# Yeicor/sdf-viewer

Measured on AMD Instinct MI355X. Metric: Mvoxels/s grid fill + Mrays/s sphere-trace @1080p, demo SDF, higher is better.
Workload: dtype f32

## Files before the change

### profiles/r02/raymarch_loop_hand.s

```
s_mov_b64 s[76:77], exec
s_and_b64 exec, exec, s[2:3]
s_cbranch_execz .Ldone_2
v_mov_b32 v40, v9
v_mov_b32 v42, v14
v_mov_b32 v43, v15
v_mov_b32 v44, v1
v_mov_b32 v46, v2
v_mov_b32 v47, v3
s_mov_b32 s66, s5
s_mov_b32 s67, s6
s_mov_b32 s70, s17
s_mov_b32 s71, s18
s_mov_b32 s72, 0xbf000000
s_mov_b32 s73, 0xbf000000
s_add_i32 s75, s40, -1
s_add_i32 s82, s19, 2
s_add_i32 s83, s19, 4
s_movk_i32 s74, 254
s_lshl_b32 s64, 1, s82
s_add_i32 s86, s23, s82
s_lshl_b32 s86, 1, s86
s_add_u32 s68, s34, s86
s_addc_u32 s69, s35, 0
s_add_u32 s64, s34, s64
s_addc_u32 s65, s35, 0
s_add_u32 s86, s64, s86
s_addc_u32 s87, s65, 0
v_mov_b32 v68, 0x7f800000
v_mov_b32 v70, 0x7f800000
v_mov_b32 v71, 0x7f800000
.Lloop_2:
v_max3_f32 v32, |v40|, |v42|, |v43|
v_subrev_f32_e32 v48, s4, v40
v_pk_add_f32 v[50:51], v[42:43], s[66:67] neg_lo:[0,1] neg_hi:[0,1]
v_mul_f32_e32 v48, s16, v48
v_pk_mul_f32 v[50:51], v[50:51], s[70:71]
v_subrev_f32_e32 v32, s7, v32
v_add_f32_e32 v48, -0.5, v48
v_pk_add_f32 v[50:51], v[50:51], s[72:73]
v_cmpx_nlt_f32_e32 vcc, 0x38d1b717, v32
s_cbranch_execz .Ldone_2
v_sub_f32_e32 v52, v48, v68
v_sub_f32_e32 v54, v50, v70
v_sub_f32_e32 v56, v51, v71
v_max3_u32 v32, v52, v54, v56
v_cmp_gt_u32_e32 vcc, 0x3f800000, v32
s_andn1_saveexec_b64 s[78:79], vcc
s_cbranch_execnz .Lfetch_2
.Lcached_2:
s_mov_b64 exec, s[78:79]
v_sub_f32_e32 v53, 1.0, v52
v_sub_f32_e32 v55, 1.0, v54
v_sub_f32_e32 v57, 1.0, v56
v_pk_mul_f32 v[34:35], v[62:63], v[52:53] op_sel_hi:[1,0]
v_pk_mul_f32 v[38:39], v[66:67], v[52:53] op_sel_hi:[1,0]
v_pk_mul_f32 v[32:33], v[60:61], v[52:53] op_sel:[0,1] op_sel_hi:[1,1]
v_pk_mul_f32 v[36:37], v[64:65], v[52:53] op_sel:[0,1] op_sel_hi:[1,1]
v_pk_add_f32 v[32:33], v[32:33], v[34:35]
v_pk_add_f32 v[36:37], v[36:37], v[38:39]
v_pk_mul_f32 v[32:33], v[32:33], v[54:55] op_sel:[0,1] op_sel_hi:[1,1]
v_pk_mul_f32 v[36:37], v[36:37], v[54:55] op_sel_hi:[1,0]
v_pk_add_f32 v[32:33], v[32:33], v[36:37]
v_pk_mul_f32 v[32:33], v[32:33], v[56:57] op_sel:[0,1] op_sel_hi:[1,0]
v_add_f32_e32 v36, v32, v33
v_add_f32_e32 v36, 0xbdcccccd, v36
v_cmpx_ngt_f32_e32 vcc, 0x3727c5ac, v36
v_mul_f32_e32 v32, v44, v36
v_pk_mul_f32 v[34:35], v[46:47], v[36:37] op_sel_hi:[1,0]
v_add_f32_e32 v40, v40, v32
v_pk_add_f32 v[42:43], v[42:43], v[34:35]
s_add_u32 s74, s74, -1
s_cbranch_scc1 .Lloop_2
s_branch .Ldone_2
.Lfetch_2:
v_floor_f32_e32 v68, v48
v_floor_f32_e32 v70, v50
v_floor_f32_e32 v71, v51
v_cvt_i32_f32_e32 v32, v68
v_cvt_i32_f32_e32 v33, v70
v_cvt_i32_f32_e32 v34, v71
v_sub_f32_e32 v52, v48, v68
v_sub_f32_e32 v54, v50, v70
v_sub_f32_e32 v56, v51, v71
v_max3_u32 v35, v32, v33, v34
v_cmp_gt_u32_e32 vcc, s28, v35
s_xor_b64 vcc, vcc, exec
s_cbranch_scc1 .Lborder_2
v_lshl_add_u32 v39, v34, s23, v33
v_lshl_add_u32 v39, v39, s19, v32
v_lshlrev_b32_e32 v39, 2, v39
global_load_dwordx2 v[24:25], v39, s[34:35]
global_load_dwordx2 v[26:27], v39, s[64:65]
global_load_dwordx2 v[28:29], v39, s[68:69]
global_load_dwordx2 v[30:31], v39, s[86:87]
s_waitcnt vmcnt(1)
v_pk_mov_b32 v[60:61], v[24:25], v[28:29] op_sel:[0,0]
v_pk_mov_b32 v[62:63], v[24:25], v[28:29] op_sel:[1,1]
s_waitcnt vmcnt(0)
v_pk_mov_b32 v[64:65], v[26:27], v[30:31] op_sel:[0,0]
v_pk_mov_b32 v[66:67], v[26:27], v[30:31] op_sel:[1,1]
s_branch .Lcached_2
.Lborder_2:
v_max_i32_e32 v35, 0, v32
v_max_i32_e32 v37, 0, v33
v_max_i32_e32 v38, 0, v34
v_add_u32_e32 v32, 1, v32
v_add_u32_e32 v33, 1, v33
v_add_u32_e32 v34, 1, v34
v_min_i32_e32 v32, s40, v32
v_min_i32_e32 v33, s41, v33
v_min_i32_e32 v34, s42, v34
v_lshl_add_u32 v28, v38, s23, v37
v_lshl_add_u32 v29, v38, s23, v33
v_lshl_add_u32 v30, v34, s23, v37
v_lshl_add_u32 v31, v34, s23, v33
v_min_i32_e32 v36, s75, v35
v_lshlrev_b32_e32 v39, 2, v36
v_lshl_add_u32 v28, v28, s82, v39
v_lshl_add_u32 v29, v29, s82, v39
v_lshl_add_u32 v30, v30, s82, v39
v_lshl_add_u32 v31, v31, s82, v39
global_load_dwordx2 v[24:25], v28, s[34:35]
global_load_dwordx2 v[26:27], v29, s[34:35]
global_load_dwordx2 v[28:29], v30, s[34:35]
global_load_dwordx2 v[30:31], v31, s[34:35]
v_cmp_eq_u32_e64 s[80:81], v35, v36
v_add_u32_e32 v36, 1, v36
v_cmp_eq_u32_e32 vcc, v32, v36
s_waitcnt vmcnt(3)
v_cndmask_b32_e64 v60, v25, v24, s[80:81]
v_cndmask_b32_e32 v62, v24, v25, vcc
s_waitcnt vmcnt(2)
v_cndmask_b32_e64 v64, v27, v26, s[80:81]
v_cndmask_b32_e32 v66, v26, v27, vcc
s_waitcnt vmcnt(1)
v_cndmask_b32_e64 v61, v29, v28, s[80:81]
v_cndmask_b32_e32 v63, v28, v29, vcc
s_waitcnt vmcnt(0)
v_cndmask_b32_e64 v65, v31, v30, s[80:81]
v_cndmask_b32_e32 v67, v30, v31, vcc
s_branch .Lcached_2
.Ldone_2:
s_mov_b64 s[30:31], exec
s_mov_b32 s14, s74
s_and_b64 exec, s[76:77], s[2:3]
v_mov_b32 v9, v40
v_mov_b32 v14, v42
v_mov_b32 v15, v43
s_mov_b64 exec, s[76:77]
```

### sdf-viewer_amd/csrc/march_asm_loop.h

```cpp
#pragma once

#include "march_sampler.h"

namespace sdfv {
namespace {

#ifdef SDFV_TUNING
#define SDFV_MARCH_ASM_TUNE(x) x
#else
#define SDFV_MARCH_ASM_TUNE(x) ""
#endif
#define SDFV_MARCH_ASM_HEAD(ROW_BYTES)                                                                                         \
    "s_mov_b64 s[76:77], exec\n"                                                                                    \
    "s_and_b64 exec, exec, %[cov]\n"                                                                                \
    "s_cbranch_execz .Ldone_%=\n"                                                                                   \
          \
    "s_mov_b32 s66, %[miny]\n s_mov_b32 s67, %[minz]\n"                                            \
    "s_mov_b32 s70, %[ky]\n s_mov_b32 s71, %[kz]\n"                                                    \
    "s_mov_b32 s72, 0xbf000000\n s_mov_b32 s73, 0xbf000000\n"                                      \
    "s_add_i32 s75, %[wm1], -1\n"                                                                         \
    "s_lshl_b32 s82, %[w], 2\n s_lshl_b32 s83, %[w], 4\n"         \
    "s_lshl_b32 s85, %[w], 3\n"                                      \
    "s_movk_i32 s74, 254\n"                                                                      \
     \
    "s_mov_b32 s64, " ROW_BYTES "\n"                                                                                 \
    "s_mul_i32 s86, %[h], " ROW_BYTES "\n"                                                                           \
    "s_add_u32 s68, %[base_lo], s86\n s_addc_u32 s69, %[base_hi], 0\n"                                      \
    "s_add_u32 s64, %[base_lo], s64\n s_addc_u32 s65, %[base_hi], 0\n"                                      \
    "s_add_u32 s86, s64, s86\n s_addc_u32 s87, s65, 0\n"                                                    \
    SDFV_MARCH_ASM_TUNE("s_mov_b32 s84, 0\n")                  \
    "v_mov_b32 v68, 0x7f800000\n v_mov_b32 v70, 0x7f800000\n v_mov_b32 v71, 0x7f800000\n"     \
    ".Lloop_%=:\n"
#define SDFV_MARCH_ASM_OOB4_A "v_sub_f32_e64 v32, |v40|, %[mx]\n"
#define SDFV_MARCH_ASM_OOB4_B "v_sub_f32_e64 v33, |v42|, %[my]\n"
#define SDFV_MARCH_ASM_OOB4_C "v_sub_f32_e64 v34, |v43|, %[mz]\n"
#define SDFV_MARCH_ASM_OOB4_D "v_max3_f32 v32, v32, v33, v34\n"
#define SDFV_MARCH_ASM_OOB2_A "v_max3_f32 v32, |v40|, |v42|, |v43|\n"
#define SDFV_MARCH_ASM_OOB2_D "v_subrev_f32_e32 v32, %[mx], v32\n"
#define SDFV_MARCH_ASM_TOP(T_STEP, OOB_A, OOB_B, OOB_C, OOB_D)                                                      \
    OOB_A                                                                                                           \
    "v_subrev_f32_e32 v48, %[minx], v40\n"                                                                          \
    OOB_B                                                                                                           \
    "v_pk_add_f32 v[50:51], v[42:43], s[66:67] neg_lo:[0,1] neg_hi:[0,1]\n"                                         \
    OOB_C                                                                                                           \
    "v_mul_f32_e32 v48, %[kx], v48\n"                                                                               \
    "v_pk_mul_f32 v[50:51], v[50:51], s[70:71]\n"                                                                   \
    OOB_D                                                                                                           \
    "v_add_f32_e32 v48, -0.5, v48\n"                                                                                \
    "v_pk_add_f32 v[50:51], v[50:51], s[72:73]\n"                                                                   \
    "v_cmpx_nlt_f32_e32 vcc, 0x38d1b717, v32\n"                                           \
    "s_cbranch_execz .Ldone_%=\n"                                                                                   \
    "v_sub_f32_e32 v52, v48, v68\n"                                                                              \
    "v_sub_f32_e32 v54, v50, v70\n"                                                                              \
    "v_sub_f32_e32 v56, v51, v71\n" T_STEP                                                                       \
    "v_max3_u32 v32, v52, v54, v56\n"                                                                            \
    "v_cmp_gt_u32_e32 vcc, 0x3f800000, v32\n"                                                                       \
    "s_andn1_saveexec_b64 s[78:79], vcc\n"                                      \
    "s_cbranch_execnz .Lfetch_%=\n"                                  \
    ".Lcached_%=:\n"
#define SDFV_MARCH_ASM_FETCH_PREP(INTERIOR)                                                                         \
    ".Lfetch_%=:\n"                                                                                                 \
    SDFV_MARCH_ASM_TUNE("s_add_u32 s84, s84, 1\n")                                                                  \
        \
    "v_floor_f32_e32 v68, v48\n v_floor_f32_e32 v70, v50\n v_floor_f32_e32 v71, v51\n"                         \
    "v_cvt_i32_f32_e32 v32, v68\n v_cvt_i32_f32_e32 v33, v70\n v_cvt_i32_f32_e32 v34, v71\n"                      \
    "v_sub_f32_e32 v52, v48, v68\n v_sub_f32_e32 v54, v50, v70\n v_sub_f32_e32 v56, v51, v71\n"             \
     \
    "v_max3_u32 v35, v32, v33, v34\n"                                                                               \
    "v_cmp_gt_u32_e32 vcc, %[thresh], v35\n"                                                                        \
    "s_xor_b64 vcc, vcc, exec\n"                                                                                    \
    "s_cbranch_scc1 .Lborder_%=\n"                                                                                  \
    "v_mad_u32_u24 v39, v34, %[h], v33\n"                     \
    "v_mad_u32_u24 v39, v39, %[w], v32\n" INTERIOR                                                               \
    "s_branch .Lcached_%=\n"                                                                                        \
    ".Lborder_%=:\n"                                                                                                \
    "v_max_i32_e32 v35, 0, v32\n v_max_i32_e32 v37, 0, v33\n v_max_i32_e32 v38, 0, v34\n"         \
    "v_add_u32_e32 v32, 1, v32\n v_add_u32_e32 v33, 1, v33\n v_add_u32_e32 v34, 1, v34\n"                            \
    "v_min_i32_e32 v32, %[wm1], v32\n v_min_i32_e32 v33, %[hm1], v33\n v_min_i32_e32 v34, %[dm1], v34\n"   \
    "v_mad_u32_u24 v28, v38, %[h], v37\n"                                                      \
    "v_mad_u32_u24 v29, v38, %[h], v33\n"                                                      \
    "v_mad_u32_u24 v30, v34, %[h], v37\n"                                                      \
    "v_mad_u32_u24 v31, v34, %[h], v33\n"
#define SDFV_MARCH_ASM_INTERIOR_DIST                                                                                \
    "v_lshlrev_b32_e32 v39, 2, v39\n"                                                                               \
    "global_load_dwordx2 v[24:25], v39, %[base]\n"                                        \
    "global_load_dwordx2 v[26:27], v39, s[64:65]\n"                                       \
    "global_load_dwordx2 v[28:29], v39, s[68:69]\n"                                       \
    "global_load_dwordx2 v[30:31], v39, s[86:87]\n"                                       \
    "s_waitcnt vmcnt(1)\n"                                                                                          \
    "v_pk_mov_b32 v[60:61], v[24:25], v[28:29] op_sel:[0,0]\n"                                    \
    "v_pk_mov_b32 v[62:63], v[24:25], v[28:29] op_sel:[1,1]\n"                                    \
    "s_waitcnt vmcnt(0)\n"                                                                                          \
    "v_pk_mov_b32 v[64:65], v[26:27], v[30:31] op_sel:[0,0]\n"                                    \
    "v_pk_mov_b32 v[66:67], v[26:27], v[30:31] op_sel:[1,1]\n"
#define SDFV_MARCH_ASM_INTERIOR_TEX0                                                                                \
    "v_lshlrev_b32_e32 v39, 4, v39\n"                                                                               \
    "global_load_dword v60, v39, %[base]\n global_load_dword v62, v39, %[base] offset:16\n"                       \
    "global_load_dword v64, v39, s[64:65]\n global_load_dword v66, v39, s[64:65] offset:16\n"                     \
    "global_load_dword v61, v39, s[68:69]\n global_load_dword v63, v39, s[68:69] offset:16\n"                     \
    "global_load_dword v65, v39, s[86:87]\n global_load_dword v67, v39, s[86:87] offset:16\n"                     \
    "s_waitcnt vmcnt(0)\n"
#define SDFV_MARCH_ASM_INTERIOR_PAIRS                                                                               \
    "v_lshlrev_b32_e32 v39, 3, v39\n"                                                                               \
    "global_load_dwordx4 v[24:27], v39, %[base]\n"                                  \
    "global_load_dwordx4 v[28:31], v39, s[68:69]\n"                                 \
    "s_waitcnt vmcnt(0)\n"                                                                                          \
    "v_pk_mov_b32 v[60:61], v[24:25], v[28:29] op_sel:[0,0]\n"                                    \
    "v_pk_mov_b32 v[64:65], v[24:25], v[28:29] op_sel:[1,1]\n"                                    \
    "v_pk_mov_b32 v[62:63], v[26:27], v[30:31] op_sel:[0,0]\n"                                    \
    "v_pk_mov_b32 v[66:67], v[26:27], v[30:31] op_sel:[1,1]\n"
#define SDFV_MARCH_ASM_FETCH_PAIRS                                                                                  \
    "v_lshlrev_b32_e32 v35, 3, v35\n v_lshlrev_b32_e32 v32, 3, v32\n"                  \
    "v_mad_u32_u24 v24, v28, s85, v35\n v_mad_u32_u24 v25, v28, s85, v32\n"                                          \
    "global_load_dword v60, v24, %[base]\n global_load_dword v62, v25, %[base]\n"                                  \
    "v_mad_u32_u24 v26, v29, s85, v35\n v_mad_u32_u24 v27, v29, s85, v32\n"                                          \
    "global_load_dword v64, v26, %[base]\n global_load_dword v66, v27, %[base]\n"                                  \
    "v_mad_u32_u24 v24, v30, s85, v35\n v_mad_u32_u24 v25, v30, s85, v32\n"                                          \
    "global_load_dword v61, v24, %[base]\n global_load_dword v63, v25, %[base]\n"                                  \
    "v_mad_u32_u24 v26, v31, s85, v35\n v_mad_u32_u24 v27, v31, s85, v32\n"                                          \
    "global_load_dword v65, v26, %[base]\n global_load_dword v67, v27, %[base]\n"                                  \
    "s_waitcnt vmcnt(0)\n"                                                                                          \
    "s_branch .Lcached_%=\n"
#define SDFV_MARCH_ASM_INTERIOR_ILV                                                                                 \
    "s_lshr_b32 s80, %[h], 1\n"                                                                                     \
    "v_and_b32_e32 v48, 1, v33\n"                                                                  \
    "v_lshrrev_b32_e32 v35, 1, v33\n"                                                              \
    "v_add_u32_e32 v36, 1, v33\n"                                                                                   \
    "v_lshrrev_b32_e32 v36, 1, v36\n"                                                        \
    "v_mad_u32_u24 v35, v34, s80, v35\n v_mad_u32_u24 v36, v34, s80, v36\n"              \
    "v_mad_u32_u24 v35, v35, %[w], v32\n v_mad_u32_u24 v37, v36, %[w], v32\n"                                        \
    "v_lshlrev_b32_e32 v36, 3, v35\n v_lshlrev_b32_e32 v37, 3, v37\n"                                               \
    "v_cmp_eq_u32_e32 vcc, 1, v48\n"                                                                                \
    "global_load_dwordx4 v[24:27], v36, %[base]\n"                      \
    "global_load_dwordx4 v[32:35], v36, s[68:69]\n"                                                      \
    "s_and_saveexec_b64 s[80:81], vcc\n"                      \
    "global_load_dwordx3 v[28:30], v37, %[base]\n"                                   \
    "global_load_dwordx3 v[36:38], v37, s[68:69]\n"                                                      \
    "s_mov_b64 exec, s[80:81]\n"                                                                                    \
    "s_waitcnt vmcnt(2)\n"                                                                                          \
    "v_cndmask_b32_e32 v60, v24, v25, vcc\n v_cndmask_b32_e32 v62, v26, v27, vcc\n"          \
    "v_cndmask_b32_e32 v61, v32, v33, vcc\n v_cndmask_b32_e32 v63, v34, v35, vcc\n"                  \
    "s_waitcnt vmcnt(0)\n"                                                                                          \
    "v_cndmask_b32_e32 v64, v25, v28, vcc\n v_cndmask_b32_e32 v66, v27, v30, vcc\n"      \
    "v_cndmask_b32_e32 v65, v33, v36, vcc\n v_cndmask_b32_e32 v67, v35, v38, vcc\n"
#define SDFV_MARCH_ASM_ILV_ROW(R)                             \
    "v_and_b32_e32 v36, 1, v" #R "\n"                                                                     \
    "v_lshrrev_b32_e32 v" #R ", 1, v" #R "\n"                                     \
    "v_mul_u32_u24_e32 v" #R ", s85, v" #R "\n"                                                         \
    "v_lshl_add_u32 v" #R ", v36, 2, v" #R "\n"
#define SDFV_MARCH_ASM_FETCH_ILV                                                                                    \
    "v_lshlrev_b32_e32 v35, 3, v35\n v_lshlrev_b32_e32 v32, 3, v32\n"         \
    SDFV_MARCH_ASM_ILV_ROW(28) SDFV_MARCH_ASM_ILV_ROW(29) SDFV_MARCH_ASM_ILV_ROW(30) SDFV_MARCH_ASM_ILV_ROW(31)       \
    "v_add_u32_e32 v24, v28, v35\n v_add_u32_e32 v25, v28, v32\n"                                                    \
    "global_load_dword v60, v24, %[base]\n global_load_dword v62, v25, %[base]\n"                                  \
    "v_add_u32_e32 v26, v29, v35\n v_add_u32_e32 v27, v29, v32\n"                                                    \
    "global_load_dword v64, v26, %[base]\n global_load_dword v66, v27, %[base]\n"                                  \
    "v_add_u32_e32 v24, v30, v35\n v_add_u32_e32 v25, v30, v32\n"                                                    \
    "global_load_dword v61, v24, %[base]\n global_load_dword v63, v25, %[base]\n"                                  \
    "v_add_u32_e32 v26, v31, v35\n v_add_u32_e32 v27, v31, v32\n"                                                    \
    "global_load_dword v65, v26, %[base]\n global_load_dword v67, v27, %[base]\n"                                  \
    "s_waitcnt vmcnt(0)\n"                                                                                          \
    "s_branch .Lcached_%=\n"
#define SDFV_MARCH_ASM_FETCH_DIST                                                                                   \
    "v_min_i32_e32 v36, s75, v35\n"                                                         \
    "v_lshlrev_b32_e32 v39, 2, v36\n"                                                                               \
    "v_mad_u32_u24 v28, v28, s82, v39\n v_mad_u32_u24 v29, v29, s82, v39\n"                                          \
    "v_mad_u32_u24 v30, v30, s82, v39\n v_mad_u32_u24 v31, v31, s82, v39\n"                                          \
    "global_load_dwordx2 v[24:25], v28, %[base]\n"                                                     \
    "global_load_dwordx2 v[26:27], v29, %[base]\n"                                                     \
    "global_load_dwordx2 v[28:29], v30, %[base]\n"                                                     \
    "global_load_dwordx2 v[30:31], v31, %[base]\n"                                                     \
    "v_cmp_eq_u32_e64 s[80:81], v35, v36\n"                                                             \
    "v_add_u32_e32 v36, 1, v36\n"                                                                                   \
    "v_cmp_eq_u32_e32 vcc, v32, v36\n"                                                                  \
    "s_waitcnt vmcnt(3)\n"                                                                                          \
    "v_cndmask_b32_e64 v60, v25, v24, s[80:81]\n v_cndmask_b32_e32 v62, v24, v25, vcc\n"           \
    "s_waitcnt vmcnt(2)\n"                                                                                          \
    "v_cndmask_b32_e64 v64, v27, v26, s[80:81]\n v_cndmask_b32_e32 v66, v26, v27, vcc\n"           \
    "s_waitcnt vmcnt(1)\n"                                                                                          \
    "v_cndmask_b32_e64 v61, v29, v28, s[80:81]\n v_cndmask_b32_e32 v63, v28, v29, vcc\n"           \
    "s_waitcnt vmcnt(0)\n"                                                                                          \
    "v_cndmask_b32_e64 v65, v31, v30, s[80:81]\n v_cndmask_b32_e32 v67, v30, v31, vcc\n"           \
    "s_branch .Lcached_%=\n"
#define SDFV_MARCH_ASM_FETCH_TEX0                                                                                   \
    "v_lshlrev_b32_e32 v35, 4, v35\n v_lshlrev_b32_e32 v32, 4, v32\n"                  \
    "v_mad_u32_u24 v24, v28, s83, v35\n v_mad_u32_u24 v25, v28, s83, v32\n"                                          \
    "global_load_dword v60, v24, %[base]\n global_load_dword v62, v25, %[base]\n"                                  \
    "v_mad_u32_u24 v26, v29, s83, v35\n v_mad_u32_u24 v27, v29, s83, v32\n"                                          \
    "global_load_dword v64, v26, %[base]\n global_load_dword v66, v27, %[base]\n"                                  \
    "v_mad_u32_u24 v24, v30, s83, v35\n v_mad_u32_u24 v25, v30, s83, v32\n"                                          \
    "global_load_dword v61, v24, %[base]\n global_load_dword v63, v25, %[base]\n"                                  \
    "v_mad_u32_u24 v26, v31, s83, v35\n v_mad_u32_u24 v27, v31, s83, v32\n"                                          \
    "global_load_dword v65, v26, %[base]\n global_load_dword v67, v27, %[base]\n"                                  \
    "s_waitcnt vmcnt(0)\n"                                                                                          \
    "s_branch .Lcached_%=\n"
#define SDFV_MARCH_ASM_FILTER                                                                                       \
    "s_mov_b64 exec, s[78:79]\n"                                                                                    \
    "v_sub_f32_e32 v53, 1.0, v52\n v_sub_f32_e32 v55, 1.0, v54\n v_sub_f32_e32 v57, 1.0, v56\n"                \
                                                                \
    "v_pk_mul_f32 v[34:35], v[62:63], v[52:53] op_sel_hi:[1,0]\n"                                                \
    "v_pk_mul_f32 v[38:39], v[66:67], v[52:53] op_sel_hi:[1,0]\n"                                                \
    "v_pk_mul_f32 v[32:33], v[60:61], v[52:53] op_sel:[0,1] op_sel_hi:[1,1]\n"                                   \
    "v_pk_mul_f32 v[36:37], v[64:65], v[52:53] op_sel:[0,1] op_sel_hi:[1,1]\n"                                   \
    "v_pk_add_f32 v[32:33], v[32:33], v[34:35]\n"                                                    \
    "v_pk_add_f32 v[36:37], v[36:37], v[38:39]\n"                                                    \
                                                                                                   \
    "v_pk_mul_f32 v[32:33], v[32:33], v[54:55] op_sel:[0,1] op_sel_hi:[1,1]\n"                                     \
    "v_pk_mul_f32 v[36:37], v[36:37], v[54:55] op_sel_hi:[1,0]\n"                                                  \
    "v_pk_add_f32 v[32:33], v[32:33], v[36:37]\n"                                                      \
                                                                       \
    "v_pk_mul_f32 v[32:33], v[32:33], v[56:57] op_sel:[0,1] op_sel_hi:[1,0]\n"       \
    "v_add_f32_e32 v36, v32, v33\n"                                                                                 \
    "v_add_f32_e32 v36, 0xbdcccccd, v36\n"                                                                          \
                                                                                 \
    "v_cmpx_ngt_f32_e32 vcc, 0x3727c5ac, v36\n"
#define SDFV_MARCH_ASM_ADVANCE                                                                                      \
                                                           \
    "v_mul_f32_e32 v32, v44, v36\n"                                                                                \
    "v_pk_mul_f32 v[34:35], v[46:47], v[36:37] op_sel_hi:[1,0]\n"                                                  \
    "v_add_f32_e32 v40, v40, v32\n"                                                                                 \
    "v_pk_add_f32 v[42:43], v[42:43], v[34:35]\n"                                                                   \
    "s_add_u32 s74, s74, -1\n"                                                    \
    "s_cbranch_scc1 .Lloop_%=\n"                                                                                    \
    "s_branch .Ldone_%=\n"
#define SDFV_MARCH_ASM_EPILOGUE                                                                                     \
    ".Ldone_%=:\n"                                                                                                  \
    "s_mov_b64 %[ran], exec\n"                                        \
    "s_mov_b32 %[left], s74\n"                                                                                      \
    SDFV_MARCH_ASM_TUNE("s_lshl_b32 s84, s84, 16\n s_and_b32 %[left], %[left], 0xffff\n s_or_b32 %[left], %[left], s84\n") \
    "s_and_b64 exec, s[76:77], %[cov]\n"                                                                            \
    "s_nop 0\n"
#define SDFV_MARCH_ASM_END "s_mov_b64 exec, s[76:77]\n"
#define SDFV_MARCH_ASM_OPERANDS                                                                                     \
    [dx] "v"(dirx), [dy] "v"(diry), [dz] "v"(dirz), [cov] "s"(cov), [mx] "s"(a.rp.bounds_max[0]),    \
        [my] "s"(a.rp.bounds_max[1]), [mz] "s"(a.rp.bounds_max[2]), [minx] "s"(a.rp.bounds_min[0]),                 \
        [miny] "s"(a.rp.bounds_min[1]), [minz] "s"(a.rp.bounds_min[2]), [kx] "s"(kx), [ky] "s"(ky), [kz] "s"(kz),   \
        [wm1] "s"(wm1), [hm1] "s"(hm1), [dm1] "s"(dm1), [w] "s"(t.w), [h] "s"(t.h), [base] "s"(vol), [base_lo] "s"(base_lo), [base_hi] "s"(base_hi), [thresh] "s"(thresh)
#define SDFV_MARCH_ASM_CLOBBERS                                                                                     \
    "vcc", "scc", "memory", "s64", "s65", "s66", "s67", "s68", "s69", "s70", "s71", "s72", "s73", "s74", "s75",    \
        "s76", "s77", "s78", "s79", "s80", "s81", "s82", "s83", "s84", "s85", "s86", "s87", "v24", "v25", "v26", "v27", "v28",  \
        "v29", "v30", "v31", "v32", "v33", "v34", "v35", "v36", "v37", "v38", "v39", "v48", "v50", "v51", "v52",    \
        "v53", "v54", "v55", "v56", "v57", "v58", "v59", "v60", "v61", "v62", "v63", "v64", "v65", "v66", "v67", "v68",   \
        "v70", "v71"

template <int MODE, bool T>
__device__ __forceinline__ void march_asm(const RaymarchArgs& a, const Tex& t, V3 ray_dir, bool covered, V3& ray_pos,
                                          float& dist_from_origin, int& status, int& steps, int& iterations) {
    const float* __restrict__ vol = march_volume<MODE>(a);
    auto uniform = [](float f) { return __int_as_float(__builtin_amdgcn_readfirstlane(__float_as_int(f))); };
    const float kx = uniform(a.inv_bsize[0] * (float)t.w), ky = uniform(a.inv_bsize[1] * (float)t.h),
                kz = uniform(a.inv_bsize[2] * (float)t.d);
    const int wm1 = t.w - 1, hm1 = t.h - 1, dm1 = t.d - 1;
    const unsigned long long cov = __ballot(covered);
    const uint32_t base_lo = (uint32_t)(uintptr_t)vol, base_hi = (uint32_t)((uintptr_t)vol >> 32);
    const uint32_t thresh = (t.w == t.h && t.h == t.d && !a.no_interior_fetch) ? (uint32_t)t.w - 1u : 0u;
    unsigned long long ran_out;
    int left = 254;
    register float px asm("v40") = ray_pos.x;
    register float py asm("v42") = ray_pos.y;
    register float pz asm("v43") = ray_pos.z;
    register float dirx asm("v44") = ray_dir.x;
    register float diry asm("v46") = ray_dir.y;
    register float dirz asm("v47") = ray_dir.z;
#define SDFV_MARCH_ASM_OOB_BOX SDFV_MARCH_ASM_OOB4_A, SDFV_MARCH_ASM_OOB4_B, SDFV_MARCH_ASM_OOB4_C, SDFV_MARCH_ASM_OOB4_D
#define SDFV_MARCH_ASM_OOB_CUBE SDFV_MARCH_ASM_OOB2_A, "", "", SDFV_MARCH_ASM_OOB2_D
#define SDFV_MARCH_ASM_TOP_(T_STEP, ...) SDFV_MARCH_ASM_TOP(T_STEP, __VA_ARGS__)
#define SDFV_MARCH_ASM_RUN_AUX(SHIFT, INTERIOR, FETCH, OOB)                                                         \
    asm volatile("v_mov_b32 v58, %[tt]\n v_mov_b32 v59, 0\n" SDFV_MARCH_ASM_HEAD(SHIFT)                             \
                 SDFV_MARCH_ASM_TOP_("v_add_u32_e32 v59, 1, v59\n", OOB) SDFV_MARCH_ASM_FILTER                       \
                 "v_add_f32_e32 v58, v58, v36\n" SDFV_MARCH_ASM_ADVANCE SDFV_MARCH_ASM_FETCH_PREP(INTERIOR) FETCH    \
                 SDFV_MARCH_ASM_EPILOGUE "v_mov_b32 %[tt], v58\n v_mov_b32 %[n], v59\n" SDFV_MARCH_ASM_END           \
                 : [px] "+v"(px), [py] "+v"(py), [pz] "+v"(pz), [tt] "+v"(tt), [n] "+v"(n), [ran] "=&s"(ran_out),   \
                   [left] "=&s"(left)                                                                               \
                 : SDFV_MARCH_ASM_OPERANDS                                                                          \
                 : SDFV_MARCH_ASM_CLOBBERS)
#define SDFV_MARCH_ASM_RUN(SHIFT, INTERIOR, FETCH, OOB)                                                             \
    asm volatile(SDFV_MARCH_ASM_HEAD(SHIFT) SDFV_MARCH_ASM_TOP_("", OOB) SDFV_MARCH_ASM_FILTER SDFV_MARCH_ASM_ADVANCE \
                     SDFV_MARCH_ASM_FETCH_PREP(INTERIOR) FETCH SDFV_MARCH_ASM_EPILOGUE SDFV_MARCH_ASM_END            \
                 : [px] "+v"(px), [py] "+v"(py), [pz] "+v"(pz), [ran] "=&s"(ran_out), [left] "=&s"(left)            \
                 : SDFV_MARCH_ASM_OPERANDS                                                                          \
                 : SDFV_MARCH_ASM_CLOBBERS)
#define SDFV_MARCH_ASM_VOL_TEX0 "s83", SDFV_MARCH_ASM_INTERIOR_TEX0, SDFV_MARCH_ASM_FETCH_TEX0
#define SDFV_MARCH_ASM_VOL_DIST "s82", SDFV_MARCH_ASM_INTERIOR_DIST, SDFV_MARCH_ASM_FETCH_DIST
#define SDFV_MARCH_ASM_VOL_PAIRS "s85", SDFV_MARCH_ASM_INTERIOR_PAIRS, SDFV_MARCH_ASM_FETCH_PAIRS
#define SDFV_MARCH_ASM_VOL_ILV "s82", SDFV_MARCH_ASM_INTERIOR_ILV, SDFV_MARCH_ASM_FETCH_ILV
#define SDFV_MARCH_ASM_PER_BOX(RUN, ...)                                                                            \
    if (cube) RUN(__VA_ARGS__, SDFV_MARCH_ASM_OOB_CUBE);                                                            \
    else RUN(__VA_ARGS__, SDFV_MARCH_ASM_OOB_BOX)
#define SDFV_MARCH_ASM_PER_VOLUME(RUN)                                                                              \
    if (MODE == kMarchIlv) { SDFV_MARCH_ASM_PER_BOX(RUN, SDFV_MARCH_ASM_VOL_ILV); }                                 \
    else if (MODE == kMarchPairs) { SDFV_MARCH_ASM_PER_BOX(RUN, SDFV_MARCH_ASM_VOL_PAIRS); }                        \
    else if (MODE == kMarchDist) { SDFV_MARCH_ASM_PER_BOX(RUN, SDFV_MARCH_ASM_VOL_DIST); }                          \
    else { SDFV_MARCH_ASM_PER_BOX(RUN, SDFV_MARCH_ASM_VOL_TEX0); }
    const bool cube = a.cube_box != 0;
    if (T) {
        float tt = dist_from_origin;
        int n = 0;
        SDFV_MARCH_ASM_PER_VOLUME(SDFV_MARCH_ASM_RUN_AUX)
        dist_from_origin = tt;
        steps = n;
    } else {
// ... 18 lines not shown
```

Measured before the change: 204,600.

## Unroll hand-written sphere-trace loop 3x and move fetch exec masking to out-of-line blocks

The inline-asm march loop is unrolled three times, with the iteration counter cut from 254 to 84 so the total step budget stays about the same. Each copy gets its own out-of-line fetch and border block, and exit labels that reconstruct the remaining-step count when tuning is enabled. The common cached path now takes a plain vcc branch and skips the per-iteration saveexec/restore exec pair; the fetch block sets and restores exec itself. The aim is to cut loop overhead and scalar exec traffic per step, at the cost of larger code and a step budget of 252 instead of 254.

```diff
diff --git a/profiles/r02/raymarch_loop_hand.s b/profiles/r02/raymarch_loop_hand.s
--- a/profiles/r02/raymarch_loop_hand.s
+++ b/profiles/r02/raymarch_loop_hand.s
@@ -1,54 +1,120 @@
 s_mov_b64 s[76:77], exec
-s_and_b64 exec, exec, s[2:3]
-s_cbranch_execz .Ldone_2
-v_mov_b32 v40, v9
-v_mov_b32 v42, v14
-v_mov_b32 v43, v15
-v_mov_b32 v44, v1
-v_mov_b32 v46, v2
-v_mov_b32 v47, v3
+s_and_b64 exec, exec, s[12:13]
+s_cbranch_execz .Ldone_16
 s_mov_b32 s66, s5
 s_mov_b32 s67, s6
-s_mov_b32 s70, s17
-s_mov_b32 s71, s18
+s_mov_b32 s70, s23
+s_mov_b32 s71, s36
 s_mov_b32 s72, 0xbf000000
 s_mov_b32 s73, 0xbf000000
 s_add_i32 s75, s40, -1
-s_add_i32 s82, s19, 2
-s_add_i32 s83, s19, 4
-s_movk_i32 s74, 254
-s_lshl_b32 s64, 1, s82
-s_add_i32 s86, s23, s82
-s_lshl_b32 s86, 1, s86
-s_add_u32 s68, s34, s86
-s_addc_u32 s69, s35, 0
-s_add_u32 s64, s34, s64
-s_addc_u32 s65, s35, 0
+s_lshl_b32 s82, s10, 2
+s_lshl_b32 s83, s10, 4
+s_lshl_b32 s85, s10, 3
+s_movk_i32 s74, 84
+s_mov_b32 s64, s82
+s_mul_i32 s86, s38, s82
+s_add_u32 s68, s2, s86
+s_addc_u32 s69, s3, 0
+s_add_u32 s64, s2, s64
+s_addc_u32 s65, s3, 0
 s_add_u32 s86, s64, s86
 s_addc_u32 s87, s65, 0
 v_mov_b32 v68, 0x7f800000
 v_mov_b32 v70, 0x7f800000
 v_mov_b32 v71, 0x7f800000
-.Lloop_2:
+.Lloop_16:
 v_max3_f32 v32, |v40|, |v42|, |v43|
 v_subrev_f32_e32 v48, s4, v40
 v_pk_add_f32 v[50:51], v[42:43], s[66:67] neg_lo:[0,1] neg_hi:[0,1]
-v_mul_f32_e32 v48, s16, v48
+v_mul_f32_e32 v48, s22, v48
 v_pk_mul_f32 v[50:51], v[50:51], s[70:71]
 v_subrev_f32_e32 v32, s7, v32
 v_add_f32_e32 v48, -0.5, v48
 v_pk_add_f32 v[50:51], v[50:51], s[72:73]
 v_cmpx_nlt_f32_e32 vcc, 0x38d1b717, v32
-s_cbranch_execz .Ldone_2
+s_cbranch_execz .Ldone0_16
 v_sub_f32_e32 v52, v48, v68
 v_sub_f32_e32 v54, v50, v70
 v_sub_f32_e32 v56, v51, v71
 v_max3_u32 v32, v52, v54, v56
-v_cmp_gt_u32_e32 vcc, 0x3f800000, v32
-s_andn1_saveexec_b64 s[78:79], vcc
-s_cbranch_execnz .Lfetch_2
-.Lcached_2:
-s_mov_b64 exec, s[78:79]
+v_cmp_le_u32_e32 vcc, 0x3f800000, v32
+s_cbranch_vccnz .Lfetch0_16
+.Lcached0_16:
+v_sub_f32_e32 v53, 1.0, v52
+v_sub_f32_e32 v55, 1.0, v54
+v_sub_f32_e32 v57, 1.0, v56
+v_pk_mul_f32 v[34:35], v[62:63], v[52:53] op_sel_hi:[1,0]
+v_pk_mul_f32 v[38:39], v[66:67], v[52:53] op_sel_hi:[1,0]
+v_pk_mul_f32 v[32:33], v[60:61], v[52:53] op_sel:[0,1] op_sel_hi:[1,1]
+v_pk_mul_f32 v[36:37], v[64:65], v[52:53] op_sel:[0,1] op_sel_hi:[1,1]
+v_pk_add_f32 v[32:33], v[32:33], v[34:35]
+v_pk_add_f32 v[36:37], v[36:37], v[38:39]
+v_pk_mul_f32 v[32:33], v[32:33], v[54:55] op_sel:[0,1] op_sel_hi:[1,1]
+v_pk_mul_f32 v[36:37], v[36:37], v[54:55] op_sel_hi:[1,0]
+v_pk_add_f32 v[32:33], v[32:33], v[36:37]
+v_pk_mul_f32 v[32:33], v[32:33], v[56:57] op_sel:[0,1] op_sel_hi:[1,0]
+v_add_f32_e32 v36, v32, v33
+v_add_f32_e32 v36, 0xbdcccccd, v36
+v_cmpx_ngt_f32_e32 vcc, 0x3727c5ac, v36
+v_mul_f32_e32 v32, v44, v36
+v_pk_mul_f32 v[34:35], v[46:47], v[36:37] op_sel_hi:[1,0]
+v_add_f32_e32 v40, v40, v32
+v_pk_add_f32 v[42:43], v[42:43], v[34:35]
+v_max3_f32 v32, |v40|, |v42|, |v43|
+v_subrev_f32_e32 v48, s4, v40
+v_pk_add_f32 v[50:51], v[42:43], s[66:67] neg_lo:[0,1] neg_hi:[0,1]
+v_mul_f32_e32 v48, s22, v48
+v_pk_mul_f32 v[50:51], v[50:51], s[70:71]
+v_subrev_f32_e32 v32, s7, v32
+v_add_f32_e32 v48, -0.5, v48
+v_pk_add_f32 v[50:51], v[50:51], s[72:73]
+v_cmpx_nlt_f32_e32 vcc, 0x38d1b717, v32
+s_cbranch_execz .Ldone1_16
+v_sub_f32_e32 v52, v48, v68
+v_sub_f32_e32 v54, v50, v70
+v_sub_f32_e32 v56, v51, v71
+v_max3_u32 v32, v52, v54, v56
+v_cmp_le_u32_e32 vcc, 0x3f800000, v32
+s_cbranch_vccnz .Lfetch1_16
+.Lcached1_16:
+v_sub_f32_e32 v53, 1.0, v52
+v_sub_f32_e32 v55, 1.0, v54
+v_sub_f32_e32 v57, 1.0, v56
+v_pk_mul_f32 v[34:35], v[62:63], v[52:53] op_sel_hi:[1,0]
+v_pk_mul_f32 v[38:39], v[66:67], v[52:53] op_sel_hi:[1,0]
+v_pk_mul_f32 v[32:33], v[60:61], v[52:53] op_sel:[0,1] op_sel_hi:[1,1]
+v_pk_mul_f32 v[36:37], v[64:65], v[52:53] op_sel:[0,1] op_sel_hi:[1,1]
+v_pk_add_f32 v[32:33], v[32:33], v[34:35]
+v_pk_add_f32 v[36:37], v[36:37], v[38:39]
+v_pk_mul_f32 v[32:33], v[32:33], v[54:55] op_sel:[0,1] op_sel_hi:[1,1]
+v_pk_mul_f32 v[36:37], v[36:37], v[54:55] op_sel_hi:[1,0]
+v_pk_add_f32 v[32:33], v[32:33], v[36:37]
+v_pk_mul_f32 v[32:33], v[32:33], v[56:57] op_sel:[0,1] op_sel_hi:[1,0]
+v_add_f32_e32 v36, v32, v33
+v_add_f32_e32 v36, 0xbdcccccd, v36
+v_cmpx_ngt_f32_e32 vcc, 0x3727c5ac, v36
+v_mul_f32_e32 v32, v44, v36
+v_pk_mul_f32 v[34:35], v[46:47], v[36:37] op_sel_hi:[1,0]
+v_add_f32_e32 v40, v40, v32
+v_pk_add_f32 v[42:43], v[42:43], v[34:35]
+v_max3_f32 v32, |v40|, |v42|, |v43|
+v_subrev_f32_e32 v48, s4, v40
+v_pk_add_f32 v[50:51], v[42:43], s[66:67] neg_lo:[0,1] neg_hi:[0,1]
+v_mul_f32_e32 v48, s22, v48
+v_pk_mul_f32 v[50:51], v[50:51], s[70:71]
+v_subrev_f32_e32 v32, s7, v32
+v_add_f32_e32 v48, -0.5, v48
+v_pk_add_f32 v[50:51], v[50:51], s[72:73]
+v_cmpx_nlt_f32_e32 vcc, 0x38d1b717, v32
+s_cbranch_execz .Ldone2_16
+v_sub_f32_e32 v52, v48, v68
+v_sub_f32_e32 v54, v50, v70
+v_sub_f32_e32 v56, v51, v71
+v_max3_u32 v32, v52, v54, v56
+v_cmp_le_u32_e32 vcc, 0x3f800000, v32
+s_cbranch_vccnz .Lfetch2_16
+.Lcached2_16:
 v_sub_f32_e32 v53, 1.0, v52
 v_sub_f32_e32 v55, 1.0, v54
 v_sub_f32_e32 v57, 1.0, v56
@@ -70,9 +136,10 @@
 v_add_f32_e32 v40, v40, v32
 v_pk_add_f32 v[42:43], v[42:43], v[34:35]
 s_add_u32 s74, s74, -1
-s_cbranch_scc1 .Lloop_2
-s_branch .Ldone_2
-.Lfetch_2:
+s_cbranch_scc1 .Lloop_16
+s_branch .Ldone_16
+.Lfetch0_16:
+s_and_saveexec_b64 s[78:79], vcc
 v_floor_f32_e32 v68, v48
 v_floor_f32_e32 v70, v50
 v_floor_f32_e32 v71, v51
@@ -83,13 +150,13 @@
 v_sub_f32_e32 v54, v50, v70
 v_sub_f32_e32 v56, v51, v71
 v_max3_u32 v35, v32, v33, v34
-v_cmp_gt_u32_e32 vcc, s28, v35
+v_cmp_gt_u32_e32 vcc, s37, v35
 s_xor_b64 vcc, vcc, exec
-s_cbranch_scc1 .Lborder_2
-v_lshl_add_u32 v39, v34, s23, v33
-v_lshl_add_u32 v39, v39, s19, v32
+s_cbranch_scc1 .Lborder0_16
+v_mad_u32_u24 v39, v34, s38, v33
+v_mad_u32_u24 v39, v39, s10, v32
 v_lshlrev_b32_e32 v39, 2, v39
-global_load_dwordx2 v[24:25], v39, s[34:35]
+global_load_dwordx2 v[24:25], v39, s[2:3]
 global_load_dwordx2 v[26:27], v39, s[64:65]
 global_load_dwordx2 v[28:29], v39, s[68:69]
 global_load_dwordx2 v[30:31], v39, s[86:87]
@@ -99,8 +166,9 @@
 s_waitcnt vmcnt(0)
 v_pk_mov_b32 v[64:65], v[26:27], v[30:31] op_sel:[0,0]
 v_pk_mov_b32 v[66:67], v[26:27], v[30:31] op_sel:[1,1]
-s_branch .Lcached_2
-.Lborder_2:
+s_mov_b64 exec, s[78:79]
+s_branch .Lcached0_16
+.Lborder0_16:
 v_max_i32_e32 v35, 0, v32
 v_max_i32_e32 v37, 0, v33
 v_max_i32_e32 v38, 0, v34
@@ -108,22 +176,22 @@
 v_add_u32_e32 v33, 1, v33
 v_add_u32_e32 v34, 1, v34
 v_min_i32_e32 v32, s40, v32
-v_min_i32_e32 v33, s41, v33
-v_min_i32_e32 v34, s42, v34
-v_lshl_add_u32 v28, v38, s23, v37
-v_lshl_add_u32 v29, v38, s23, v33
-v_lshl_add_u32 v30, v34, s23, v37
-v_lshl_add_u32 v31, v34, s23, v33
+v_min_i32_e32 v33, s33, v33
+v_min_i32_e32 v34, s19, v34
+v_mad_u32_u24 v28, v38, s38, v37
+v_mad_u32_u24 v29, v38, s38, v33
+v_mad_u32_u24 v30, v34, s38, v37
+v_mad_u32_u24 v31, v34, s38, v33
 v_min_i32_e32 v36, s75, v35
 v_lshlrev_b32_e32 v39, 2, v36
-v_lshl_add_u32 v28, v28, s82, v39
-v_lshl_add_u32 v29, v29, s82, v39
-v_lshl_add_u32 v30, v30, s82, v39
-v_lshl_add_u32 v31, v31, s82, v39
-global_load_dwordx2 v[24:25], v28, s[34:35]
-global_load_dwordx2 v[26:27], v29, s[34:35]
-global_load_dwordx2 v[28:29], v30, s[34:35]
-global_load_dwordx2 v[30:31], v31, s[34:35]
+v_mad_u32_u24 v28, v28, s82, v39
+v_mad_u32_u24 v29, v29, s82, v39
+v_mad_u32_u24 v30, v30, s82, v39
+v_mad_u32_u24 v31, v31, s82, v39
+global_load_dwordx2 v[24:25], v28, s[2:3]
+global_load_dwordx2 v[26:27], v29, s[2:3]
+global_load_dwordx2 v[28:29], v30, s[2:3]
+global_load_dwordx2 v[30:31], v31, s[2:3]
 v_cmp_eq_u32_e64 s[80:81], v35, v36
 v_add_u32_e32 v36, 1, v36
 v_cmp_eq_u32_e32 vcc, v32, v36
@@ -139,12 +207,156 @@
 s_waitcnt vmcnt(0)
 v_cndmask_b32_e64 v65, v31, v30, s[80:81]
 v_cndmask_b32_e32 v67, v30, v31, vcc
-s_branch .Lcached_2
-.Ldone_2:
-s_mov_b64 s[30:31], exec
-s_mov_b32 s14, s74
-s_and_b64 exec, s[76:77], s[2:3]
-v_mov_b32 v9, v40
-v_mov_b32 v14, v42
-v_mov_b32 v15, v43
+s_mov_b64 exec, s[78:79]
+s_branch .Lcached0_16
+.Lfetch1_16:
+s_and_saveexec_b64 s[78:79], vcc
+v_floor_f32_e32 v68, v48
+v_floor_f32_e32 v70, v50
+v_floor_f32_e32 v71, v51
+v_cvt_i32_f32_e32 v32, v68
+v_cvt_i32_f32_e32 v33, v70
+v_cvt_i32_f32_e32 v34, v71
+v_sub_f32_e32 v52, v48, v68
+v_sub_f32_e32 v54, v50, v70
+v_sub_f32_e32 v56, v51, v71
+v_max3_u32 v35, v32, v33, v34
+v_cmp_gt_u32_e32 vcc, s37, v35
+s_xor_b64 vcc, vcc, exec
+s_cbranch_scc1 .Lborder1_16
+v_mad_u32_u24 v39, v34, s38, v33
+v_mad_u32_u24 v39, v39, s10, v32
+v_lshlrev_b32_e32 v39, 2, v39
+global_load_dwordx2 v[24:25], v39, s[2:3]
+global_load_dwordx2 v[26:27], v39, s[64:65]
+global_load_dwordx2 v[28:29], v39, s[68:69]
+global_load_dwordx2 v[30:31], v39, s[86:87]
+s_waitcnt vmcnt(1)
+v_pk_mov_b32 v[60:61], v[24:25], v[28:29] op_sel:[0,0]
+v_pk_mov_b32 v[62:63], v[24:25], v[28:29] op_sel:[1,1]
+s_waitcnt vmcnt(0)
+v_pk_mov_b32 v[64:65], v[26:27], v[30:31] op_sel:[0,0]
+v_pk_mov_b32 v[66:67], v[26:27], v[30:31] op_sel:[1,1]
+s_mov_b64 exec, s[78:79]
+s_branch .Lcached1_16
+.Lborder1_16:
+v_max_i32_e32 v35, 0, v32
+v_max_i32_e32 v37, 0, v33
+v_max_i32_e32 v38, 0, v34
+v_add_u32_e32 v32, 1, v32
+v_add_u32_e32 v33, 1, v33
+v_add_u32_e32 v34, 1, v34
+v_min_i32_e32 v32, s40, v32
+v_min_i32_e32 v33, s33, v33
+v_min_i32_e32 v34, s19, v34
+v_mad_u32_u24 v28, v38, s38, v37
+v_mad_u32_u24 v29, v38, s38, v33
+v_mad_u32_u24 v30, v34, s38, v37
+v_mad_u32_u24 v31, v34, s38, v33
+v_min_i32_e32 v36, s75, v35
+v_lshlrev_b32_e32 v39, 2, v36
+v_mad_u32_u24 v28, v28, s82, v39
+v_mad_u32_u24 v29, v29, s82, v39
+v_mad_u32_u24 v30, v30, s82, v39
+v_mad_u32_u24 v31, v31, s82, v39
+global_load_dwordx2 v[24:25], v28, s[2:3]
+global_load_dwordx2 v[26:27], v29, s[2:3]
+global_load_dwordx2 v[28:29], v30, s[2:3]
+global_load_dwordx2 v[30:31], v31, s[2:3]
+v_cmp_eq_u32_e64 s[80:81], v35, v36
+v_add_u32_e32 v36, 1, v36
+v_cmp_eq_u32_e32 vcc, v32, v36
+s_waitcnt vmcnt(3)
+v_cndmask_b32_e64 v60, v25, v24, s[80:81]
+v_cndmask_b32_e32 v62, v24, v25, vcc
+s_waitcnt vmcnt(2)
+v_cndmask_b32_e64 v64, v27, v26, s[80:81]
+v_cndmask_b32_e32 v66, v26, v27, vcc
+s_waitcnt vmcnt(1)
+v_cndmask_b32_e64 v61, v29, v28, s[80:81]
+v_cndmask_b32_e32 v63, v28, v29, vcc
+s_waitcnt vmcnt(0)
+v_cndmask_b32_e64 v65, v31, v30, s[80:81]
+v_cndmask_b32_e32 v67, v30, v31, vcc
+s_mov_b64 exec, s[78:79]
+s_branch .Lcached1_16
+.Lfetch2_16:
+s_and_saveexec_b64 s[78:79], vcc
+v_floor_f32_e32 v68, v48
+v_floor_f32_e32 v70, v50
+v_floor_f32_e32 v71, v51
+v_cvt_i32_f32_e32 v32, v68
+v_cvt_i32_f32_e32 v33, v70
+v_cvt_i32_f32_e32 v34, v71
+v_sub_f32_e32 v52, v48, v68
+v_sub_f32_e32 v54, v50, v70
+v_sub_f32_e32 v56, v51, v71
+v_max3_u32 v35, v32, v33, v34
+v_cmp_gt_u32_e32 vcc, s37, v35
+s_xor_b64 vcc, vcc, exec
+s_cbranch_scc1 .Lborder2_16
+v_mad_u32_u24 v39, v34, s38, v33
+v_mad_u32_u24 v39, v39, s10, v32
+v_lshlrev_b32_e32 v39, 2, v39
+global_load_dwordx2 v[24:25], v39, s[2:3]
+global_load_dwordx2 v[26:27], v39, s[64:65]
+global_load_dwordx2 v[28:29], v39, s[68:69]
+global_load_dwordx2 v[30:31], v39, s[86:87]
+s_waitcnt vmcnt(1)
+v_pk_mov_b32 v[60:61], v[24:25], v[28:29] op_sel:[0,0]
+v_pk_mov_b32 v[62:63], v[24:25], v[28:29] op_sel:[1,1]
+s_waitcnt vmcnt(0)
+v_pk_mov_b32 v[64:65], v[26:27], v[30:31] op_sel:[0,0]
+v_pk_mov_b32 v[66:67], v[26:27], v[30:31] op_sel:[1,1]
+s_mov_b64 exec, s[78:79]
+s_branch .Lcached2_16
+.Lborder2_16:
+v_max_i32_e32 v35, 0, v32
+v_max_i32_e32 v37, 0, v33
+v_max_i32_e32 v38, 0, v34
+v_add_u32_e32 v32, 1, v32
+v_add_u32_e32 v33, 1, v33
+v_add_u32_e32 v34, 1, v34
+v_min_i32_e32 v32, s40, v32
+v_min_i32_e32 v33, s33, v33
+v_min_i32_e32 v34, s19, v34
+v_mad_u32_u24 v28, v38, s38, v37
+v_mad_u32_u24 v29, v38, s38, v33
+v_mad_u32_u24 v30, v34, s38, v37
+v_mad_u32_u24 v31, v34, s38, v33
+v_min_i32_e32 v36, s75, v35
+v_lshlrev_b32_e32 v39, 2, v36
+v_mad_u32_u24 v28, v28, s82, v39
+v_mad_u32_u24 v29, v29, s82, v39
+v_mad_u32_u24 v30, v30, s82, v39
+v_mad_u32_u24 v31, v31, s82, v39
+global_load_dwordx2 v[24:25], v28, s[2:3]
+global_load_dwordx2 v[26:27], v29, s[2:3]
+global_load_dwordx2 v[28:29], v30, s[2:3]
+global_load_dwordx2 v[30:31], v31, s[2:3]
+v_cmp_eq_u32_e64 s[80:81], v35, v36
+v_add_u32_e32 v36, 1, v36
+v_cmp_eq_u32_e32 vcc, v32, v36
+s_waitcnt vmcnt(3)
+v_cndmask_b32_e64 v60, v25, v24, s[80:81]
+v_cndmask_b32_e32 v62, v24, v25, vcc
+s_waitcnt vmcnt(2)
+v_cndmask_b32_e64 v64, v27, v26, s[80:81]
+v_cndmask_b32_e32 v66, v26, v27, vcc
+s_waitcnt vmcnt(1)
+v_cndmask_b32_e64 v61, v29, v28, s[80:81]
+v_cndmask_b32_e32 v63, v28, v29, vcc
+s_waitcnt vmcnt(0)
+v_cndmask_b32_e64 v65, v31, v30, s[80:81]
+v_cndmask_b32_e32 v67, v30, v31, vcc
+s_mov_b64 exec, s[78:79]
+s_branch .Lcached2_16
+.Ldone0_16:
+.Ldone1_16:
+.Ldone2_16:
+.Ldone_16:
+s_mov_b64 s[42:43], exec
+s_mov_b32 s20, s74
+s_and_b64 exec, s[76:77], s[12:13]
+s_nop 0
 s_mov_b64 exec, s[76:77]
diff --git a/sdf-viewer_amd/csrc/march_asm_loop.h b/sdf-viewer_amd/csrc/march_asm_loop.h
--- a/sdf-viewer_amd/csrc/march_asm_loop.h
+++ b/sdf-viewer_amd/csrc/march_asm_loop.h
@@ -10,7 +10,7 @@
 #else
 #define SDFV_MARCH_ASM_TUNE(x) ""
 #endif
-#define SDFV_MARCH_ASM_HEAD(ROW_BYTES)                                                                                         \
+#define SDFV_MARCH_ASM_HEAD(ROW_BYTES)                                                                                        \
     "s_mov_b64 s[76:77], exec\n"                                                                                    \
     "s_and_b64 exec, exec, %[cov]\n"                                                                                \
     "s_cbranch_execz .Ldone_%=\n"                                                                                   \
@@ -21,7 +21,7 @@
     "s_add_i32 s75, %[wm1], -1\n"                                                                         \
     "s_lshl_b32 s82, %[w], 2\n s_lshl_b32 s83, %[w], 4\n"         \
     "s_lshl_b32 s85, %[w], 3\n"                                      \
-    "s_movk_i32 s74, 254\n"                                                                      \
+    "s_movk_i32 s74, 84\n"                                                         \
      \
     "s_mov_b32 s64, " ROW_BYTES "\n"                                                                                 \
     "s_mul_i32 s86, %[h], " ROW_BYTES "\n"                                                                           \
@@ -37,7 +37,7 @@
 #define SDFV_MARCH_ASM_OOB4_D "v_max3_f32 v32, v32, v33, v34\n"
 #define SDFV_MARCH_ASM_OOB2_A "v_max3_f32 v32, |v40|, |v42|, |v43|\n"
 #define SDFV_MARCH_ASM_OOB2_D "v_subrev_f32_e32 v32, %[mx], v32\n"
-#define SDFV_MARCH_ASM_TOP(T_STEP, OOB_A, OOB_B, OOB_C, OOB_D)                                                      \
+#define SDFV_MARCH_ASM_TOP(C, T_STEP, OOB_A, OOB_B, OOB_C, OOB_D)                                                   \
     OOB_A                                                                                                           \
     "v_subrev_f32_e32 v48, %[minx], v40\n"                                                                          \
     OOB_B                                                                                                           \
@@ -49,18 +49,18 @@
     "v_add_f32_e32 v48, -0.5, v48\n"                                                                                \
     "v_pk_add_f32 v[50:51], v[50:51], s[72:73]\n"                                                                   \
     "v_cmpx_nlt_f32_e32 vcc, 0x38d1b717, v32\n"                                           \
-    "s_cbranch_execz .Ldone_%=\n"                                                                                   \
+    "s_cbranch_execz .Ldone" C "_%=\n"                                                                              \
     "v_sub_f32_e32 v52, v48, v68\n"                                                                              \
     "v_sub_f32_e32 v54, v50, v70\n"                                                                              \
     "v_sub_f32_e32 v56, v51, v71\n" T_STEP                                                                       \
     "v_max3_u32 v32, v52, v54, v56\n"                                                                            \
-    "v_cmp_gt_u32_e32 vcc, 0x3f800000, v32\n"                                                                       \
-    "s_andn1_saveexec_b64 s[78:79], vcc\n"                                      \
-    "s_cbranch_execnz .Lfetch_%=\n"                                  \
-    ".Lcached_%=:\n"
-#define SDFV_MARCH_ASM_FETCH_PREP(INTERIOR)                                                                         \
-    ".Lfetch_%=:\n"                                                                                                 \
+    "v_cmp_le_u32_e32 vcc, 0x3f800000, v32\n"                                    \
+    "s_cbranch_vccnz .Lfetch" C "_%=\n"                              \
+    ".Lcached" C "_%=:\n"
+#define SDFV_MARCH_ASM_FETCH_BLOCK(C, INTERIOR, BORDER)                                                             \
+    ".Lfetch" C "_%=:\n"                                                                                            \
     SDFV_MARCH_ASM_TUNE("s_add_u32 s84, s84, 1\n")                                                                  \
+    "s_and_saveexec_b64 s[78:79], vcc\n"                                        \
         \
     "v_floor_f32_e32 v68, v48\n v_floor_f32_e32 v70, v50\n v_floor_f32_e32 v71, v51\n"                         \
     "v_cvt_i32_f32_e32 v32, v68\n v_cvt_i32_f32_e32 v33, v70\n v_cvt_i32_f32_e32 v34, v71\n"                      \
@@ -69,18 +69,19 @@
     "v_max3_u32 v35, v32, v33, v34\n"                                                                               \
     "v_cmp_gt_u32_e32 vcc, %[thresh], v35\n"                                                                        \
     "s_xor_b64 vcc, vcc, exec\n"                                                                                    \
-    "s_cbranch_scc1 .Lborder_%=\n"                                                                                  \
+    "s_cbranch_scc1 .Lborder" C "_%=\n"                                                                             \
     "v_mad_u32_u24 v39, v34, %[h], v33\n"                     \
     "v_mad_u32_u24 v39, v39, %[w], v32\n" INTERIOR                                                               \
-    "s_branch .Lcached_%=\n"                                                                                        \
-    ".Lborder_%=:\n"                                                                                                \
+    "s_mov_b64 exec, s[78:79]\n s_branch .Lcached" C "_%=\n"                                                       \
+    ".Lborder" C "_%=:\n"                                                                                           \
     "v_max_i32_e32 v35, 0, v32\n v_max_i32_e32 v37, 0, v33\n v_max_i32_e32 v38, 0, v34\n"         \
     "v_add_u32_e32 v32, 1, v32\n v_add_u32_e32 v33, 1, v33\n v_add_u32_e32 v34, 1, v34\n"                            \
     "v_min_i32_e32 v32, %[wm1], v32\n v_min_i32_e32 v33, %[hm1], v33\n v_min_i32_e32 v34, %[dm1], v34\n"   \
     "v_mad_u32_u24 v28, v38, %[h], v37\n"                                                      \
     "v_mad_u32_u24 v29, v38, %[h], v33\n"                                                      \
     "v_mad_u32_u24 v30, v34, %[h], v37\n"                                                      \
-    "v_mad_u32_u24 v31, v34, %[h], v33\n"
+    "v_mad_u32_u24 v31, v34, %[h], v33\n"                                                      \
+    BORDER "s_mov_b64 exec, s[78:79]\n s_branch .Lcached" C "_%=\n"
 #define SDFV_MARCH_ASM_INTERIOR_DIST                                                                                \
     "v_lshlrev_b32_e32 v39, 2, v39\n"                                                                               \
     "global_load_dwordx2 v[24:25], v39, %[base]\n"                                        \
@@ -119,8 +120,7 @@
     "global_load_dword v61, v24, %[base]\n global_load_dword v63, v25, %[base]\n"                                  \
     "v_mad_u32_u24 v26, v31, s85, v35\n v_mad_u32_u24 v27, v31, s85, v32\n"                                          \
     "global_load_dword v65, v26, %[base]\n global_load_dword v67, v27, %[base]\n"                                  \
-    "s_waitcnt vmcnt(0)\n"                                                                                          \
-    "s_branch .Lcached_%=\n"
+    "s_waitcnt vmcnt(0)\n"
 #define SDFV_MARCH_ASM_INTERIOR_ILV                                                                                 \
     "s_lshr_b32 s80, %[h], 1\n"                                                                                     \
     "v_and_b32_e32 v48, 1, v33\n"                                                                  \
@@ -159,8 +159,7 @@
     "global_load_dword v61, v24, %[base]\n global_load_dword v63, v25, %[base]\n"                                  \
     "v_add_u32_e32 v26, v31, v35\n v_add_u32_e32 v27, v31, v32\n"                                                    \
     "global_load_dword v65, v26, %[base]\n global_load_dword v67, v27, %[base]\n"                                  \
-    "s_waitcnt vmcnt(0)\n"                                                                                          \
-    "s_branch .Lcached_%=\n"
+    "s_waitcnt vmcnt(0)\n"
 #define SDFV_MARCH_ASM_FETCH_DIST                                                                                   \
     "v_min_i32_e32 v36, s75, v35\n"                                                         \
     "v_lshlrev_b32_e32 v39, 2, v36\n"                                                                               \
@@ -180,8 +179,7 @@
     "s_waitcnt vmcnt(1)\n"                                                                                          \
     "v_cndmask_b32_e64 v61, v29, v28, s[80:81]\n v_cndmask_b32_e32 v63, v28, v29, vcc\n"           \
     "s_waitcnt vmcnt(0)\n"                                                                                          \
-    "v_cndmask_b32_e64 v65, v31, v30, s[80:81]\n v_cndmask_b32_e32 v67, v30, v31, vcc\n"           \
-    "s_branch .Lcached_%=\n"
+    "v_cndmask_b32_e64 v65, v31, v30, s[80:81]\n v_cndmask_b32_e32 v67, v30, v31, vcc\n"
 #define SDFV_MARCH_ASM_FETCH_TEX0                                                                                   \
     "v_lshlrev_b32_e32 v35, 4, v35\n v_lshlrev_b32_e32 v32, 4, v32\n"                  \
     "v_mad_u32_u24 v24, v28, s83, v35\n v_mad_u32_u24 v25, v28, s83, v32\n"                                          \
@@ -192,10 +190,8 @@
     "global_load_dword v61, v24, %[base]\n global_load_dword v63, v25, %[base]\n"                                  \
     "v_mad_u32_u24 v26, v31, s83, v35\n v_mad_u32_u24 v27, v31, s83, v32\n"                                          \
     "global_load_dword v65, v26, %[base]\n global_load_dword v67, v27, %[base]\n"                                  \
-    "s_waitcnt vmcnt(0)\n"                                                                                          \
-    "s_branch .Lcached_%=\n"
+    "s_waitcnt vmcnt(0)\n"
 #define SDFV_MARCH_ASM_FILTER                                                                                       \
-    "s_mov_b64 exec, s[78:79]\n"                                                                                    \
     "v_sub_f32_e32 v53, 1.0, v52\n v_sub_f32_e32 v55, 1.0, v54\n v_sub_f32_e32 v57, 1.0, v56\n"                \
                                                                 \
     "v_pk_mul_f32 v[34:35], v[62:63], v[52:53] op_sel_hi:[1,0]\n"                                                \
@@ -219,11 +215,13 @@
     "v_mul_f32_e32 v32, v44, v36\n"                                                                                \
     "v_pk_mul_f32 v[34:35], v[46:47], v[36:37] op_sel_hi:[1,0]\n"                                                  \
     "v_add_f32_e32 v40, v40, v32\n"                                                                                 \
-    "v_pk_add_f32 v[42:43], v[42:43], v[34:35]\n"                                                                   \
-    "s_add_u32 s74, s74, -1\n"                                                    \
+    "v_pk_add_f32 v[42:43], v[42:43], v[34:35]\n"
+#define SDFV_MARCH_ASM_LOOP_BACK                                                                                    \
+    "s_add_u32 s74, s74, -1\n"                                                         \
     "s_cbranch_scc1 .Lloop_%=\n"                                                                                    \
     "s_branch .Ldone_%=\n"
 #define SDFV_MARCH_ASM_EPILOGUE                                                                                     \
+    SDFV_MARCH_ASM_EXITS                                                                                            \
     ".Ldone_%=:\n"                                                                                                  \
     "s_mov_b64 %[ran], exec\n"                                        \
     "s_mov_b32 %[left], s74\n"                                                                                      \
@@ -264,19 +262,31 @@
     register float dirz asm("v47") = ray_dir.z;
 #define SDFV_MARCH_ASM_OOB_BOX SDFV_MARCH_ASM_OOB4_A, SDFV_MARCH_ASM_OOB4_B, SDFV_MARCH_ASM_OOB4_C, SDFV_MARCH_ASM_OOB4_D
 #define SDFV_MARCH_ASM_OOB_CUBE SDFV_MARCH_ASM_OOB2_A, "", "", SDFV_MARCH_ASM_OOB2_D
-#define SDFV_MARCH_ASM_TOP_(T_STEP, ...) SDFV_MARCH_ASM_TOP(T_STEP, __VA_ARGS__)
+#define SDFV_MARCH_ASM_TOP_(C, T_STEP, ...) SDFV_MARCH_ASM_TOP(C, T_STEP, __VA_ARGS__)
+#define SDFV_MARCH_ASM_ITER(C, T_STEP, T_ACC, ...)                                                                  \
+    SDFV_MARCH_ASM_TOP_(C, T_STEP, __VA_ARGS__) SDFV_MARCH_ASM_FILTER T_ACC SDFV_MARCH_ASM_ADVANCE
+#define SDFV_MARCH_ASM_LOOP(T_STEP, T_ACC, ...)                                                                   \
+    SDFV_MARCH_ASM_ITER("0", T_STEP, T_ACC, __VA_ARGS__) SDFV_MARCH_ASM_ITER("1", T_STEP, T_ACC, __VA_ARGS__)       \
+    SDFV_MARCH_ASM_ITER("2", T_STEP, T_ACC, __VA_ARGS__) SDFV_MARCH_ASM_LOOP_BACK
+#define SDFV_MARCH_ASM_FETCH_BLOCKS(INTERIOR, BORDER)                                                               \
+    SDFV_MARCH_ASM_FETCH_BLOCK("0", INTERIOR, BORDER) SDFV_MARCH_ASM_FETCH_BLOCK("1", INTERIOR, BORDER)             \
+    SDFV_MARCH_ASM_FETCH_BLOCK("2", INTERIOR, BORDER)
+#define SDFV_MARCH_ASM_EXITS                                                                                        \
+    ".Ldone0_%=:\n" SDFV_MARCH_ASM_TUNE("s_mul_i32 s74, s74, 3\n s_add_u32 s74, s74, 2\n s_branch .Ldone_%=\n")     \
+    ".Ldone1_%=:\n" SDFV_MARCH_ASM_TUNE("s_mul_i32 s74, s74, 3\n s_add_u32 s74, s74, 1\n s_branch .Ldone_%=\n")     \
+    ".Ldone2_%=:\n" SDFV_MARCH_ASM_TUNE("s_mul_i32 s74, s74, 3\n")
 #define SDFV_MARCH_ASM_RUN_AUX(SHIFT, INTERIOR, FETCH, OOB)                                                         \
     asm volatile("v_mov_b32 v58, %[tt]\n v_mov_b32 v59, 0\n" SDFV_MARCH_ASM_HEAD(SHIFT)                             \
-                 SDFV_MARCH_ASM_TOP_("v_add_u32_e32 v59, 1, v59\n", OOB) SDFV_MARCH_ASM_FILTER                       \
-                 "v_add_f32_e32 v58, v58, v36\n" SDFV_MARCH_ASM_ADVANCE SDFV_MARCH_ASM_FETCH_PREP(INTERIOR) FETCH    \
+                 SDFV_MARCH_ASM_LOOP("v_add_u32_e32 v59, 1, v59\n", "v_add_f32_e32 v58, v58, v36\n", OOB)           \
+                 SDFV_MARCH_ASM_FETCH_BLOCKS(INTERIOR, FETCH)                                                       \
                  SDFV_MARCH_ASM_EPILOGUE "v_mov_b32 %[tt], v58\n v_mov_b32 %[n], v59\n" SDFV_MARCH_ASM_END           \
                  : [px] "+v"(px), [py] "+v"(py), [pz] "+v"(pz), [tt] "+v"(tt), [n] "+v"(n), [ran] "=&s"(ran_out),   \
                    [left] "=&s"(left)                                                                               \
                  : SDFV_MARCH_ASM_OPERANDS                                                                          \
                  : SDFV_MARCH_ASM_CLOBBERS)
 #define SDFV_MARCH_ASM_RUN(SHIFT, INTERIOR, FETCH, OOB)                                                             \
-    asm volatile(SDFV_MARCH_ASM_HEAD(SHIFT) SDFV_MARCH_ASM_TOP_("", OOB) SDFV_MARCH_ASM_FILTER SDFV_MARCH_ASM_ADVANCE \
-                     SDFV_MARCH_ASM_FETCH_PREP(INTERIOR) FETCH SDFV_MARCH_ASM_EPILOGUE SDFV_MARCH_ASM_END            \
+    asm volatile(SDFV_MARCH_ASM_HEAD(SHIFT) SDFV_MARCH_ASM_LOOP("", "", OOB)                                        \
+                     SDFV_MARCH_ASM_FETCH_BLOCKS(INTERIOR, FETCH) SDFV_MARCH_ASM_EPILOGUE SDFV_MARCH_ASM_END         \
                  : [px] "+v"(px), [py] "+v"(py), [pz] "+v"(pz), [ran] "=&s"(ran_out), [left] "=&s"(left)            \
                  : SDFV_MARCH_ASM_OPERANDS                                                                          \
                  : SDFV_MARCH_ASM_CLOBBERS)
```

Result: no change. 204,600 (-0.0%).
